# EDIpack/EDIpack

Measured on AMD Instinct MI355X. Metric: Lanczos H*v iterations/sec, largest (Nup,Ndw) sector, higher is better.
Workload: dtype f64

## Files before the change

edipack_amd/capi.py:

```python
from __future__ import annotations

import ctypes as C
import os

import numpy as np

HERE = os.path.dirname(os.path.abspath(__file__))
LIB_PATH = os.environ.get("EDIGPU_LIB", os.path.join(HERE, "lib", "libedigpu.so"))
HEADER_PATH = os.path.join(os.path.dirname(HERE), "include", "edigpu.h")

MAXORB = 5
MAXSUNDRY = 64
MAXBATH = 16


class EdigpuError(RuntimeError):
    """Raised when a C-ABI call returns non-zero (the Fortran shim does ``stop msg``)."""


class EdigpuModel(C.Structure):
    _fields_ = [
        ("ed_mode", C.c_int32), ("bath_type", C.c_int32),
        ("norb", C.c_int32), ("nbath", C.c_int32), ("nspin", C.c_int32), ("hfmode", C.c_int32),
        ("xmu", C.c_double),
        ("uloc", C.c_double * MAXORB),
        ("ust", C.c_double * (MAXORB * MAXORB)),
        ("jh", C.c_double * (MAXORB * MAXORB)),
        ("jx", C.c_double * (MAXORB * MAXORB)),
        ("jp", C.c_double * (MAXORB * MAXORB)),
        ("hloc", C.c_double * (2 * 2 * MAXORB * MAXORB * 2)),
        ("pair_field", C.c_double * MAXORB),
        ("be", C.c_double * (2 * MAXORB * MAXBATH)),
        ("bv", C.c_double * (2 * MAXORB * MAXBATH)),
        ("bd", C.c_double * (2 * MAXORB * MAXBATH)),
        ("bu", C.c_double * (2 * MAXORB * MAXBATH)),
        ("hb", C.c_double * (2 * 2 * MAXORB * MAXORB * MAXBATH * 2)),
        ("nph", C.c_int32), ("pad_", C.c_int32),
        ("w0_ph", C.c_double), ("a_ph", C.c_double),
        ("g_ph", C.c_double * (MAXORB * MAXORB)),
        ("spin_field", C.c_double * (MAXORB * 3)),
        ("exc_field", C.c_double * 4),
        ("nsundry", C.c_int32),
        ("pad2_", C.c_int32),
        ("sundry_op", C.c_int32 * (MAXSUNDRY * 8)),
        ("sundry_u", C.c_double * MAXSUNDRY),
    ]


_lib = None

_vp = C.c_void_p
_i64 = C.c_int64
_pi64 = C.POINTER(C.c_int64)
_pi32 = C.POINTER(C.c_int32)
_pd = C.POINTER(C.c_double)
_pint = C.POINTER(C.c_int)

SIGNATURES = {
    "edigpu_last_error": (C.c_char_p, []),
    "edigpu_version": (C.c_int, []),
    "edigpu_image_info": (C.c_int, [C.c_void_p, C.POINTER(C.c_int32)]),
    "edigpu_model_sizeof": (C.c_int64, []),
    "edigpu_device_count": (C.c_int, [_pint]),
    "edigpu_init": (C.c_int, [C.c_int]),
    "edigpu_normal_create": (C.c_int, [C.POINTER(_vp), _i64, _i64, _i64, _i64, _pd, _pi64, _pi32, _pd,
                                       _pi64, _pi32, _pd, _pi64, _pi32, _pd]),
    "edigpu_csr_create_d": (C.c_int, [C.POINTER(_vp), _i64, _i64, _i64, _pi64, _pi32, _pd]),
    "edigpu_csr_create_z": (C.c_int, [C.POINTER(_vp), _i64, _i64, _i64, _pi64, _pi32, _pd]),
    "edigpu_normal_build": (C.c_int, [C.POINTER(_vp), C.POINTER(EdigpuModel), C.c_int, C.c_int, _i64, _i64]),
    "edigpu_normal_build_z": (C.c_int, [C.POINTER(_vp), C.POINTER(EdigpuModel), C.c_int, C.c_int]),
    "edigpu_flat_build": (C.c_int, [C.POINTER(_vp), C.POINTER(EdigpuModel), C.c_int, _i64, _i64]),
    "edigpu_flat_build_jz": (C.c_int, [C.POINTER(_vp), C.POINTER(EdigpuModel), C.c_int, C.c_int, _i64, _i64]),
    "edigpu_direct_build_jz": (C.c_int, [C.POINTER(_vp), C.POINTER(EdigpuModel), C.c_int, C.c_int, _i64, _i64]),
    "edigpu_sector_map_jz": (C.c_int, [_vp, C.c_int, C.c_int, _pi32, _pi64]),
    "edigpu_direct_build": (C.c_int, [C.POINTER(_vp), C.POINTER(EdigpuModel), C.c_int, _i64, _i64]),
    "edigpu_sector_dim": (C.c_int, [C.POINTER(EdigpuModel), C.c_int, C.c_int, _pi64]),
    "edigpu_info": (C.c_int, [_vp, _pi64]),
    "edigpu_algorithmic_bytes": (C.c_int, [_vp, _pd, _pd]),
    "edigpu_normal_export": (C.c_int, [_vp, _pd, _pi64, _pi32, _pd, _pi64, _pi32, _pd, _pi64, _pi32, _pd]),
    "edigpu_csr_export": (C.c_int, [_vp, _pi64, _pi32, _pd]),
    "edigpu_apply_d": (C.c_int, [_vp, _i64, _pd, _pd]),
    "edigpu_apply_z": (C.c_int, [_vp, _i64, _pd, _pd]),
    "edigpu_apply_dev": (C.c_int, [_vp, _vp, _vp, _vp]),
    "edigpu_apply_local_dev": (C.c_int, [_vp, _vp, _vp, _vp]),
    "edigpu_apply_remote_dev": (C.c_int, [_vp, _vp, _vp, _vp]),
    "edigpu_normal_transpose_info": (C.c_int, [_vp, C.POINTER(C.c_int32)]),
    "edigpu_normal_apply_rows_dev": (C.c_int, [_vp, _i64, _i64, _vp, _vp, _vp]),
    "edigpu_normal_apply_cols_dev": (C.c_int, [_vp, _i64, _i64, _i64, C.c_int32, _vp, _vp, _vp]),
    "edigpu_transpose_pack": (C.c_int, [_i64, _i64, _i64, C.c_int32, _i64, C.c_int32, _vp, _vp, _vp]),
    "edigpu_transpose_unpack_add": (C.c_int, [_i64, _i64, _i64, C.c_int32, _i64, C.c_int32, _vp, _vp, _vp]),
    "edigpu_transpose_rotate_pack": (C.c_int, [C.c_int32, _i64, _i64, _i64, C.c_int32, _i64, C.c_int32, _vp, _vp, _vp,
                                               _vp, _vp]),
    "edigpu_transpose_unpack_add_dot2": (C.c_int, [_i64, _i64, _i64, C.c_int32, _i64, C.c_int32, _vp, _vp, _vp, _vp,
                                                   _vp, _vp, _vp]),
    "edigpu_lanczos_tridiag": (C.c_int, [_vp, _pd, C.c_int, _pd, _pd, C.c_double, _pint]),
    "edigpu_lanczos_eigh": (C.c_int, [_vp, C.c_int, C.c_double, C.c_int, _pd, _pd, _pd, _pint]),
    "edigpu_orbs_build": (C.c_int, [C.POINTER(_vp), C.POINTER(EdigpuModel), _pi32, _pi32]),
    "edigpu_orbs_build_rows": (C.c_int, [C.POINTER(_vp), C.POINTER(EdigpuModel), _pi32, _pi32, _i64, _i64]),
    "edigpu_orbs_create": (C.c_int, [C.POINTER(_vp), C.c_int, _pi64, _pd, _pi64, _pi32, _pd]),
    "edigpu_lanczos_eigh_multi": (C.c_int, [_vp, C.c_int, C.c_int, C.c_double, C.c_int, _vp, _pd, _vp,
                                            C.POINTER(C.c_int), C.POINTER(C.c_int)]),
    "edigpu_apply_op_normal": (C.c_int, [_vp, _vp, _vp, _vp, C.c_int, C.c_int, C.c_int, _vp]),
    "edigpu_apply_op_flat": (C.c_int, [_vp, _vp, _vp, _vp, C.c_int, C.c_int, C.c_int, _vp]),
    "edigpu_apply_cops_normal": (C.c_int, [_vp, _vp, _vp, _vp, C.c_int, _pd, _pi32, _pi32, _pi32, _vp]),
    "edigpu_lanczos_tridiag_dev": (C.c_int, [_vp, _vp, C.c_int, _pd, _pd, C.c_double, C.POINTER(C.c_int), _pd]),
    "edigpu_vec_work_doubles": (C.c_int, []),
    "edigpu_vec_rotate": (C.c_int, [_i64, _vp, _vp, _vp, _vp]),
    "edigpu_vec_add_dot": (C.c_int, [_i64, _vp, _vp, _vp, _vp, _vp, _vp]),
    "edigpu_vec_axpy_nrm2": (C.c_int, [_i64, _vp, _vp, _vp, _vp, _vp, _vp]),
    "edigpu_vec_scale": (C.c_int, [_i64, _vp, _vp, _vp]),
    "edigpu_vec_rotate_lazy": (C.c_int, [_i64, _vp, _vp, _vp, _vp]),
    "edigpu_vec_add_dot2": (C.c_int, [_i64, _vp, _vp, _vp, _vp, _vp, _vp]),
    "edigpu_time_apply": (C.c_int, [_vp, C.c_int, C.c_int, C.c_int, _pd]),
    "edigpu_lanczos_bench": (C.c_int, [_vp, C.c_int, C.c_int, _pd, _pd]),
# ... 102 lines not shown
```

edipack_amd/csrc/edigpu_capi.hip:

```cpp
#include <algorithm>
#include <chrono>
#include <cmath>
#include <cstdlib>
#include <cstring>
#include <map>
#include <memory>
#include <mutex>
#include <tuple>

#include "host_ib.hpp"
#include "host_sb.hpp"
#include "kernels.hpp"

namespace edigpu {

static thread_local std::string g_err;
static thread_local int g_device = 0;
void set_error(const std::string& msg) { g_err = msg; }

template <class T>
static int dev_upload(T** d, const T* h, size_t n) {
  *d = nullptr;
  if (n == 0) return 0;
  EDIGPU_HIP(hipMalloc((void**)d, n * sizeof(T)));
// ... 2058 lines not shown
    set_error("edigpu_sector_map: NULL argument");
    return 1;
  }
  std::vector<int32_t> st;
  std::string e = sector_map(*model, q1, q2, which, st);
  if (!e.empty()) {
    set_error(e);
    return 1;
  }
  if (map) {
    if (*n < (int64_t)st.size()) {
      set_error("edigpu_sector_map: output buffer too small");
      return 1;
    }
    std::copy(st.begin(), st.end(), map);
  }
  *n = (int64_t)st.size();
  return 0;
}

int edigpu_sector_map_jz(const edigpu_model* model, int ntot, int twojz, int32_t* map, int64_t* n) {
  if (!model || !n) {
    set_error("edigpu_sector_map_jz: NULL argument");
    return 1;
  }
  std::vector<int32_t> st;
  std::string e = sector_map_jz(*model, ntot, twojz, st);
  if (!e.empty()) {
    set_error(e);
    return 1;
  }
  if (map) {
    if (*n < (int64_t)st.size()) {
      set_error("edigpu_sector_map_jz: output buffer too small");
      return 1;
    }
    std::copy(st.begin(), st.end(), map);
  }
  *n = (int64_t)st.size();
  return 0;
}

int edigpu_image_info(edigpu_handle s, int32_t image[6]) {
  if (!s || !image || s->kind != 0) {
    set_error("edigpu_image_info: not a normal-mode handle");
    return 1;
  }
  image[0] = s->factored;
  image[1] = s->factored ? s->fac_nterms : 0;
  image[2] = s->factored ? s->fac_nimp : 0;
  image[3] = s->panel_mode;
  image[4] = s->ib ? kIbPanel : (s->blk_shift ? (1 << s->blk_shift) : 0);
  image[5] = s->ib ? (s->ib->sb ? (s->ib->sb->nhalf == 2 ? 4 : (s->ib->pr.on ? 5 : 3)) : s->ib->nhalf) : 0;
  return 0;
}

int edigpu_info(edigpu_handle s, int64_t info[10]) {
  if (!s || !info) {
    set_error("edigpu_info: NULL argument");
    return 1;
  }
  info[0] = s->dim;
  info[1] = s->nloc;
  info[2] = s->row_first;
  info[3] = s->is_complex;
  info[4] = s->kind;
  info[5] = s->dim_up;
  info[6] = s->dim_dw;
  if (s->kind == 0) {
    info[7] = s->h_up.nnz() + s->h_dw.nnz();
    info[8] = s->nd_nnz;
  } else if (s->kind == 4) {
    info[7] = s->sub_s->h_up.nnz() + s->sub_s->h_dw.nnz();
    info[8] = s->sub_s->nd_nnz;
  } else if (s->kind == 2) {
    info[7] = s->dir_nterms;
    info[8] = 0;
  } else if (s->kind == 3) {
    info[7] = 0;
    for (const HostCsr& f : s->h_orbs_fac) info[7] += f.nnz();
    info[8] = s->orbs.naxes;
  } else {
    info[7] = s->loc.nnz;
    info[8] = s->nonloc.nnz;
  }
  info[9] = s->device;
  return 0;
}

int edigpu_algorithmic_bytes(edigpu_handle s, double* bytes_hv, double* bytes_step) {
  if (!s) {
    set_error("edigpu_algorithmic_bytes: NULL handle");
    return 1;
  }
  double b = 0.0;
  const double sz = s->is_complex ? 16.0 : 8.0;
  if (s->kind == 4) {
    const edigpu_sector* r = s->sub_s;
    const double n = (double)s->nloc;
    b = 3.0 * sz * n;
    if (r->has_nd) b += (sz + 4.0) * (double)r->nd_nnz + 4.0 * (n + 1.0);
    b += (sz + 4.0) * (double)(r->h_up.nnz() + r->h_dw.nnz()) + 4.0 * (double)(r->dim_up + r->dim_dw + 2);
  } else if (s->kind == 0) {
    const double n = (double)s->nloc;
    b = 3.0 * sz * n;
    if (s->has_nd) b += (sz + 4.0) * (double)s->nd_nnz + 4.0 * (n + 1.0);
// ... 1179 lines not shown
```

edipack_amd/csrc/kernels.hpp:

```cpp
#pragma once
#include <functional>

#include "edigpu_internal.hpp"

namespace edigpu {

enum { SC_ALPHA = 0, SC_BETA = 1, SC_STOP = 2, SC_NDONE = 3, SC_NORM = 4, SC_THR = 5, SC_EXACT = 6, SC_AB = 8 };
constexpr int kRedBlocks = 1024;
constexpr int kMaxPartials = 1 << 16;

int ensure_dynamic_lds(const void* kernel, size_t bytes);
int resident_blocks(const void* kernel, int threads, size_t dyn_lds);
int device_cu_count();

int launch_normal(const edigpu_sector* s, const double* v_local, const double* v_full, double* hv,
                  int phase, hipStream_t st);
int normal_pick_rows_per_block(int64_t dim_up, int64_t dw_count);
bool normal_transposable(const edigpu_sector* s);
bool normal_transposable_el(const edigpu_sector* s);
int launch_normal_rows(const edigpu_sector* s, int64_t dw_first, int64_t dw_count, const double* v_rows,
                       double* hv_rows, hipStream_t st);
int launch_normal_cols(const edigpu_sector* s, int64_t col_first, int64_t ncol, int64_t stride, int halo,
                       const double* w, double* hv, hipStream_t st);
int launch_eph_scatter(int64_t n, const double* t, double* up, double c_up, double* dn, double c_dn, hipStream_t st);
int launch_deinterleave(int64_t n, const double* z, double* re, double* im, hipStream_t st);
int launch_combine_interleave(int64_t n, const double* yr, const double* yi, const double* t1, const double* t2,
                              double* z, hipStream_t st);
int launch_transpose_pack(int64_t dim_up, int64_t nrows, int64_t q, int world, int64_t pcol, int halo,
                          const double* v_rows, double* send, hipStream_t st);
int launch_transpose_unpack_add(int64_t dim_up, int64_t nrows, int64_t q, int world, int64_t pcol, int halo,
                                const double* recv, double* hv_rows, hipStream_t st);
bool normal_lanczos_fusable(const edigpu_sector* s);
int launch_normal_lanczos(const edigpu_sector* s, double* P, double* Q, const double* scal,
                          double* partial, int64_t partial_cap, bool first, bool lazy_axpy, hipStream_t st, int* npartial,
                          int nlanc = 0, bool* finalized = nullptr, double* X = nullptr, bool* in_x = nullptr);
int lz_finalize_alpha_beta(const double* P, const double* Q, int64_t n, double* partial, int np,
                           double* scal, int iter, int nlanc, hipStream_t st);
int lz_finalize_alpha(const double* partial, int np, double* scal, int iter, int nlanc, hipStream_t st);

int launch_csr(const DevCsr& a, int cplx, const double* x, double* y, int accumulate,
               hipStream_t st);
int launch_zero(double* y, int64_t n, hipStream_t st);

int launch_direct_lanczos(const edigpu_sector* s, const double* v_full, double* q, double* partial, int64_t cap, int* np,
                          const double* sig, hipStream_t st);
bool csr_lanczos_fusable(const DevCsr& a);
int launch_csr_lanczos(const DevCsr& a, int cplx, const double* x, double* y, double* partial, int64_t cap, int* np,
                       const double* sig, hipStream_t st);
int lz_rotate_lazy(double* P, double* Q, int64_t n, const double* scal, hipStream_t st);
int lz_next_vector(const double* P, const double* Q, double* X, int64_t n, const double* scal, bool lazy, hipStream_t st);
int launch_direct(const edigpu_sector* s, const double* v_full, double* hv, hipStream_t st);

int lz_norm_begin(double* vin, int64_t n, double* partial, double* scal, hipStream_t st);
int lz_rotate(double* vin, double* vout, int64_t n, const double* scal, hipStream_t st);
int lz_alpha(const double* vin, double* vout, const double* tmp, int64_t n, double* partial,
             double* scal, int iter, int nlanc, hipStream_t st);
int lz_beta(const double* vin, double* vout, int64_t n, double* partial, double* scal, int iter,
            int nlanc, hipStream_t st);
int lz_axpy_coef(double* acc, const double* vin, int64_t n, double coef, const double* scal,
                 int iter, hipStream_t st);
int lz_add_dot3(const double* P, double* Q, const double* tmp, int64_t n, const double* scal, double* partial, int* np,
                hipStream_t st);
int lz_fill_random(double* v, int64_t n, uint64_t seed, hipStream_t st);
int vec_to_blocked(const double* src, double* dst, int64_t dim_up, int64_t dim_dw, int shift, hipStream_t st);
int vec_from_blocked(const double* src, double* dst, int64_t dim_up, int64_t dim_dw, int shift, hipStream_t st);
int launch_normal_blocked(const edigpu_sector* s, const double* v, double* hv, hipStream_t st);
int vec_to_ib(const IbDev* ib, const double* src, double* dst, hipStream_t st);
int vec_from_ib(const IbDev* ib, const double* src, double* dst, hipStream_t st);
int launch_ib(const edigpu_sector* s, const double* v, double* hv, hipStream_t st);
int launch_ib_lanczos(const edigpu_sector* s, const double* P, double* Q, double* X, const double* scal, double* partial,
                      int64_t partial_cap, bool first, bool lazy_axpy, hipStream_t st, int* npartial);
int launch_sb(const edigpu_sector* s, const double* v, double* hv, hipStream_t st);
int launch_normal_rows_pos(const edigpu_sector* s, const double* P, double* Q, double* X, int what, const double* scal, hipStream_t st);
int launch_sb_lanczos(const edigpu_sector* s, const double* P, double* Q, double* X, const double* scal, double* partial,
                      int64_t partial_cap, bool first, bool lazy_axpy, hipStream_t st, int* npartial);
bool sb_shardable(const edigpu_sector* s);
int sb_shard_panels(const edigpu_sector* s, int world);
int sb_shard_to_panels(const edigpu_sector* s, const double* rows, double* dst, int64_t count, int64_t q, int world, hipStream_t st);
int sb_shard_from_panels_add(const edigpu_sector* s, const double* a, const double* b, double* rows, int64_t count, int64_t q, hipStream_t st);
int launch_sb_rows_shard(const edigpu_sector* s, int64_t row0, int64_t count, int64_t q, const double* v, double* hv, hipStream_t st);
int launch_sb_cols_shard(const edigpu_sector* s, int p0, int np, int64_t q, int npmax, const double* v, double* out, hipStream_t st);
int sb_nb0(int norb);
int sb_cols_waves();
int sb_cols_gs();
size_t sb_rows_lds(int nbw, int rimg_len, bool top = false);
// ... 78 lines not shown
```

edipack_amd/csrc/kernels_normal.hip:

```cpp
#include <cstdlib>
#include <string>

#include "kernels.hpp"
#include "normal_args.hpp"

namespace edigpu {



constexpr int kE = 4;

template <bool VEC>
__device__ inline void load4(const double* __restrict__ base, int64_t i0, const bool* ok, double* out) {
  if (VEC) {
    const double2 a = ok[0] ? *reinterpret_cast<const double2*>(base + i0) : make_double2(0.0, 0.0);
    const double2 b = ok[2] ? *reinterpret_cast<const double2*>(base + i0 + 2) : make_double2(0.0, 0.0);
    out[0] = a.x;
    out[1] = a.y;
    out[2] = b.x;
    out[3] = b.y;
  } else {
#pragma unroll
    for (int e = 0; e < kE; e++) out[e] = ok[e] ? base[i0 + e] : 0.0;
  }
}

typedef const double __attribute__((address_space(3))) lds_cdouble;
__device__ inline double lds_abs_read(uint32_t byte_addr) { return *reinterpret_cast<lds_cdouble*>(byte_addr); }

template <int NT, int TD, bool USE_LDS, bool LOCAL, bool ND, bool PACKED, bool VEC, bool HDF, int FUSE,
          bool SPLIT = false>
__global__ void __launch_bounds__(NT)
    normal_rows_kernel(NormalArgs a, const double* v_local, const double* __restrict__ v_full,
                       double* hv) {
  extern __shared__ double vs[];

  const int64_t DimUp = a.dim_up;
  const int bsh = a.blk_shift;
  const int64_t bps = a.blk_ps;
  auto vix = [&](int64_t row, int64_t col) -> int64_t {
    return bsh ? (col >> bsh) * bps + (row << bsh) + (col & (((int64_t)1 << bsh) - 1)) : row * DimUp + col;
  };
  const int64_t sf = SPLIT ? a.split_first : 0, sc = SPLIT ? a.split_count : DimUp;
  const int S = ((int)sc + 2) & ~1;
  const int rowB = S * 8;
  double* coef_s = vs + (USE_LDS ? TD * S : 0);
  const int64_t r0 = (int64_t)blockIdx.x * TD;
  const int tid = threadIdx.x;
  int nr = TD;
  if (r0 + nr > a.dw_count) nr = (int)(a.dw_count - r0);
  double beta = 0.0, ibeta = 1.0;
  if (FUSE != 0) {
    if (a.scal[SC_STOP] != 0.0) return;
    if (FUSE >= 2) {
// ... 303 lines not shown
    }
    case 102: {
      auto kern = normal_rows_kernel<NT, TD, USE_LDS, true, false, PACKED, VEC, HDF, 2>;
      if (ensure_dynamic_lds((const void*)kern, lds)) return 1;
      hipLaunchKernelGGL(kern, grid, block, lds, st, a, vl, vf, hv);
      break;
    }
    case 103: {
      auto kern = normal_rows_kernel<NT, TD, USE_LDS, true, false, PACKED, VEC, HDF, 3>;
      if (ensure_dynamic_lds((const void*)kern, lds)) return 1;
      hipLaunchKernelGGL(kern, grid, block, lds, st, a, vl, vf, hv);
      break;
    }
    case 4: EDIGPU_LAUNCH_ROWS(false, true, (size_t)0, false, false, false); break;
    default: set_error("launch_normal: bad term mask"); return 1;
  }
#undef EDIGPU_LAUNCH_ROWS
  EDIGPU_HIP(hipGetLastError());
  return 0;
}

template <int TD, bool USE_LDS>
static int launch_td(const NormalArgs& a, bool packed, bool hdf, const double* vl, const double* vf,
                     double* hv, int what, hipStream_t st) {
  const bool vec = (a.dim_up % 2) == 0;
  const bool big = TD == 1 && USE_LDS && (size_t)a.dim_up * sizeof(double) > 80 * 1024;
  constexpr int NTBIG = (TD == 1 && USE_LDS) ? 1024 : 512;
#define EDIGPU_TD(PK, VC)                                                                  \
  (big ? (hdf ? launch_te<NTBIG, TD, USE_LDS, PK, VC, true>(a, vl, vf, hv, what, st)       \
              : launch_te<NTBIG, TD, USE_LDS, PK, VC, false>(a, vl, vf, hv, what, st))     \
       : (hdf ? launch_te<512, TD, USE_LDS, PK, VC, true>(a, vl, vf, hv, what, st)         \
              : launch_te<512, TD, USE_LDS, PK, VC, false>(a, vl, vf, hv, what, st)))
  if (vec) return packed ? EDIGPU_TD(true, true) : EDIGPU_TD(false, true);
  return packed ? EDIGPU_TD(true, false) : EDIGPU_TD(false, false);
#undef EDIGPU_TD
}

template <bool VEC, bool HDF>
static int launch_split_t(const edigpu_sector* s, NormalArgs a, const double* vl, double* hv, hipStream_t st) {
  constexpr int NT = 1024;
  const int64_t part = (((a.dim_up + s->row_split - 1) / s->row_split) + 1) & ~(int64_t)1;
  auto kern = normal_rows_kernel<NT, 1, true, true, false, true, VEC, HDF, 0, true>;
  const size_t lds = (size_t)((part + 2) & ~(int64_t)1) * sizeof(double) + 128 * sizeof(double);
  if (ensure_dynamic_lds((const void*)kern, lds)) return 1;
  for (int64_t first = 0; first < a.dim_up; first += part) {
    a.split_first = first;
    a.split_count = std::min<int64_t>(part, a.dim_up - first);
    hipLaunchKernelGGL(kern, dim3((unsigned)a.dw_count), dim3(NT), lds, st, a, vl, nullptr, hv);
  }
  EDIGPU_HIP(hipGetLastError());
  return 0;
}

static int launch_rows(const edigpu_sector* s, const NormalArgs& a, const double* vl,
                       const double* vf, double* hv, int what, hipStream_t st) {
  const bool packed = s->up_ell.pk != nullptr;
  const bool hdf = s->factored != 0;
  if (s->row_split > 1 && what != 4) {
    if (what != 1 && what != 5) {
      set_error("launch_normal: fused Lanczos is not available for split rows");
      return 1;
    }
    const bool vec = (a.dim_up % 2) == 0;
    const int rc = vec ? (hdf ? launch_split_t<true, true>(s, a, vl, hv, st) : launch_split_t<true, false>(s, a, vl, hv, st))
                       : (hdf ? launch_split_t<false, true>(s, a, vl, hv, st) : launch_split_t<false, false>(s, a, vl, hv, st));
    if (rc || what == 1) return rc;
    return launch_td<1, false>(a, false, hdf, vl, vf, hv, 4, st);
  }
  switch (s->rows_per_block) {
    case 0: return launch_td<1, false>(a, packed, hdf, vl, vf, hv, what, st);
    case 1: return launch_td<1, true>(a, packed, hdf, vl, vf, hv, what, st);
    case 2: return launch_td<2, true>(a, packed, hdf, vl, vf, hv, what, st);
    case 4: return launch_td<4, true>(a, packed, hdf, vl, vf, hv, what, st);
    case 8: return launch_td<8, true>(a, packed, hdf, vl, vf, hv, what, st);
    default: set_error("launch_normal: bad rows_per_block"); return 1;
  }
}

static void fill_args(const edigpu_sector* s, NormalArgs& a) {
  a.dim_up = s->dim_up;
  a.dim_dw = s->dim_dw;
  a.dw_first = s->dw_first;
  a.dw_count = s->dw_count;
  a.hd = s->d_hd;
  a.eux = s->d_eux;
  a.ed = s->d_ed;
  a.impd = s->d_impd;
  a.ell_pk = s->up_ell.pk;
  a.ell_coef = s->up_ell.coef;
  a.ell_col = s->up_ell.col;
  a.ell_val = s->up_ell.val;
  a.ell_w = s->up_ell.width;
  a.ell_typed = s->up_ell.typed;
  a.ell_pitch = s->up_ell.pitch;
  a.dw_rowptr = s->dw.rowptr32;
  a.dw_col = s->dw.col;
  a.dw_val = s->dw.val;
  a.dw_maxrow = s->dw_maxrow;
  a.nd_rp32 = s->nd.rowptr32;
  a.nd_rp64 = s->nd.wide ? s->nd.rowptr64 : nullptr;
  a.nd_col = s->nd.col;
  a.nd_val = s->nd.val;
  a.has_nd = s->has_nd;
  a.nterms = s->factored ? s->fac_nterms : 0;
  a.nd_coef = s->d_ndcoef;
  a.jup = s->d_jup;
  a.jdw = s->d_jdw;
  a.panel_mode = s->panel_mode;
  a.tile_nchunks = s->tile_nchunks;
  a.tile_rows = s->tile_rows;
// ... 170 lines not shown
```

edipack_amd/hamiltonian.py:

```python
from __future__ import annotations

import ctypes as C
from dataclasses import dataclass, field

import numpy as np

from . import capi

ED_MODES = {"normal": 0, "superc": 1, "nonsu2": 2}
BATH_TYPES = {"normal": 0, "hybrid": 1, "replica": 2, "general": 3}


@dataclass
class ImpurityModel:
    ed_mode: str = "normal"
    bath_type: str = "normal"
    norb: int = 1
    nbath: int = 1
    nspin: int = 1
    hfmode: bool = True
    xmu: float = 0.0
    uloc: np.ndarray = field(default_factory=lambda: np.zeros(1))
    ust: np.ndarray | float = 0.0
    jh: np.ndarray | float = 0.0
# ... 194 lines not shown
            rp = np.asarray(rp, dtype=np.int64)
            rps.append(rp[1:] + base)
            base += int(rp[-1])
            cols.append(np.asarray(col, dtype=np.int32))
            vals.append(np.asarray(val, dtype=np.float64))
        rp = np.ascontiguousarray(np.concatenate(rps))
        col = np.ascontiguousarray(np.concatenate(cols)) if cols else np.zeros(0, np.int32)
        val = np.ascontiguousarray(np.concatenate(vals)) if vals else np.zeros(0, np.float64)
        h = C.c_void_p()
        capi.check(capi.lib().edigpu_orbs_create(C.byref(h), len(dims), capi.pi64(dims), capi.pd(hd), capi.pi64(rp),
                                                 capi.pi32(col), capi.pd(val)), "edigpu_orbs_create")
        return cls(h)

    @classmethod
    def normal_from_arrays(cls, dim_up, dim_dw, hd, up, dw, nd=None, dw_first=0, dw_count=None):
        if dw_count is None:
            dw_count = dim_dw
        hd = np.ascontiguousarray(hd, dtype=np.float64)
        ur, uc, uv = _csr_args(*up)
        dr, dc, dv = _csr_args(*dw)
        h = C.c_void_p()
        if nd is not None:
            nr, nc, nv = _csr_args(*nd)
            args = (capi.pi64(nr), capi.pi32(nc), capi.pd(nv))
        else:
            args = (None, None, None)
        capi.check(capi.lib().edigpu_normal_create(
            C.byref(h), dim_up, dim_dw, dw_first, dw_count, capi.pd(hd),
            capi.pi64(ur), capi.pi32(uc), capi.pd(uv), capi.pi64(dr), capi.pi32(dc), capi.pd(dv), *args),
            "edigpu_normal_create")
        return cls(h)

    @classmethod
    def csr_from_arrays(cls, rowptr, col, val, ncol_global=None, row_first=0):
        cplx = np.iscomplexobj(val)
        rowptr, col, val = _csr_args(rowptr, col, val, cplx)
        nrow = rowptr.shape[0] - 1
        if ncol_global is None:
            ncol_global = nrow
        h = C.c_void_p()
        fn = capi.lib().edigpu_csr_create_z if cplx else capi.lib().edigpu_csr_create_d
        capi.check(fn(C.byref(h), nrow, ncol_global, row_first, capi.pi64(rowptr), capi.pi32(col),
                      capi.pd(val.view(np.float64))), "edigpu_csr_create")
        return cls(h)

    def vecDim(self) -> int:
        return self.nloc

    def image_info(self):
        a = (C.c_int32 * 6)()
        capi.check(capi.lib().edigpu_image_info(self._h, a), "edigpu_image_info")
        return tuple(a)

    def algorithmic_bytes(self):
        a, b = C.c_double(), C.c_double()
        capi.check(capi.lib().edigpu_algorithmic_bytes(self._h, C.byref(a), C.byref(b)))
        return a.value, b.value

    def export_normal(self):
        nup_nnz_dw = None
        L = capi.lib()
        ur = np.zeros(self.dim_up + 1, np.int64)
        dr = np.zeros(self.dim_dw + 1, np.int64)
        nr = np.zeros(self.nloc + 1, np.int64)
        capi.check(L.edigpu_normal_export(self._h, None, capi.pi64(ur), None, None, capi.pi64(dr), None, None,
                                          capi.pi64(nr), None, None))
        hd = np.zeros(self.nloc)
        uc, uv = np.zeros(ur[-1], np.int32), np.zeros(ur[-1])
        dc, dv = np.zeros(dr[-1], np.int32), np.zeros(dr[-1])
        nc, nv = np.zeros(nr[-1], np.int32), np.zeros(nr[-1])
        capi.check(L.edigpu_normal_export(self._h, capi.pd(hd), None, capi.pi32(uc), capi.pd(uv), None,
                                          capi.pi32(dc), capi.pd(dv), None, capi.pi32(nc), capi.pd(nv)))
        del nup_nnz_dw
        return hd, (ur, uc, uv), (dr, dc, dv), (nr, nc, nv)

    def export_csr(self):
        L = capi.lib()
        rp = np.zeros(self.nloc + 1, np.int64)
        nnz = self.nnz_a + self.nnz_b
        col = np.zeros(nnz, np.int32)
        val = np.zeros(nnz, self.dtype)
        capi.check(L.edigpu_csr_export(self._h, capi.pi64(rp), capi.pi32(col), capi.pd(val.view(np.float64))))
        return rp, col, val

    def apply(self, v: np.ndarray, hv: np.ndarray | None = None) -> np.ndarray:
        v = np.ascontiguousarray(v, dtype=self.dtype)
        if hv is None:
            hv = np.empty_like(v)
        fn = capi.lib().edigpu_apply_z if self.is_complex else capi.lib().edigpu_apply_d
        capi.check(fn(self._h, v.shape[0], capi.pd(v.view(np.float64)), capi.pd(hv.view(np.float64))),
                   "edigpu_apply")
        return hv

    def apply_dev(self, v_full_ptr: int, hv_ptr: int, stream: int = 0) -> None:
        capi.check(capi.lib().edigpu_apply_dev(self._h, v_full_ptr, hv_ptr, stream if stream else None), "edigpu_apply_dev")

    def apply_local_dev(self, v_local_ptr: int, hv_ptr: int, stream: int = 0) -> None:
        capi.check(capi.lib().edigpu_apply_local_dev(self._h, v_local_ptr, hv_ptr, stream if stream else None),
                   "edigpu_apply_local_dev")

    def apply_remote_dev(self, v_full_ptr: int, hv_ptr: int, stream: int = 0) -> None:
        capi.check(capi.lib().edigpu_apply_remote_dev(self._h, v_full_ptr, hv_ptr, stream if stream else None),
                   "edigpu_apply_remote_dev")

    def apply_cops_to(self, dst: "SectorHamiltonian", v_src_ptr: int, v_dst_ptr: int, coefs, creates, iorbs, ispins,
                      stream: int = 0) -> None:
# ... 213 lines not shown
```

include/edigpu.h:

```cpp
#ifndef EDIGPU_H
#define EDIGPU_H

#include <stdint.h>

#ifdef __cplusplus
extern "C" {
#endif

#define EDIGPU_MAXORB 5
#define EDIGPU_MAXSUNDRY 64
#define EDIGPU_MAXBATH 16

typedef struct edigpu_sector *edigpu_handle;

const char *edigpu_last_error(void);
int edigpu_version(void);
int64_t edigpu_model_sizeof(void);
int edigpu_device_count(int *count);
int edigpu_init(int device);

int edigpu_normal_create(edigpu_handle *h, int64_t dim_up, int64_t dim_dw, int64_t dw_first,
                         int64_t dw_count, const double *hd, const int64_t *up_rowptr,
                         const int32_t *up_col, const double *up_val, const int64_t *dw_rowptr,
                         const int32_t *dw_col, const double *dw_val, const int64_t *nd_rowptr,
// ... 13 lines not shown
  int32_t hfmode;
  double xmu;
  double uloc[EDIGPU_MAXORB];
  double ust[EDIGPU_MAXORB * EDIGPU_MAXORB];
  double jh[EDIGPU_MAXORB * EDIGPU_MAXORB];
  double jx[EDIGPU_MAXORB * EDIGPU_MAXORB];
  double jp[EDIGPU_MAXORB * EDIGPU_MAXORB];
  double hloc[2 * 2 * EDIGPU_MAXORB * EDIGPU_MAXORB * 2];
  double pair_field[EDIGPU_MAXORB];
  double be[2 * EDIGPU_MAXORB * EDIGPU_MAXBATH];
  double bv[2 * EDIGPU_MAXORB * EDIGPU_MAXBATH];
  double bd[2 * EDIGPU_MAXORB * EDIGPU_MAXBATH];
  double bu[2 * EDIGPU_MAXORB * EDIGPU_MAXBATH];
  double hb[2 * 2 * EDIGPU_MAXORB * EDIGPU_MAXORB * EDIGPU_MAXBATH * 2];
  int32_t nph;
  int32_t pad_;
  double w0_ph, a_ph;
  double g_ph[EDIGPU_MAXORB * EDIGPU_MAXORB];
  double spin_field[EDIGPU_MAXORB * 3];
  double exc_field[4];
  int32_t nsundry;
  int32_t pad2_;
  int32_t sundry_op[EDIGPU_MAXSUNDRY * 8];
  double sundry_u[EDIGPU_MAXSUNDRY];
} edigpu_model;

int edigpu_normal_build(edigpu_handle *h, const edigpu_model *model, int nup, int ndw,
                        int64_t dw_first, int64_t dw_count);
int edigpu_normal_build_z(edigpu_handle *h, const edigpu_model *model, int nup, int ndw);
int edigpu_flat_build(edigpu_handle *h, const edigpu_model *model, int sector, int64_t row_first,
                      int64_t row_count);

int edigpu_flat_build_jz(edigpu_handle *h, const edigpu_model *model, int ntot, int twojz, int64_t row_first,
                         int64_t row_count);
int edigpu_direct_build_jz(edigpu_handle *h, const edigpu_model *model, int ntot, int twojz, int64_t row_first,
                           int64_t row_count);
int edigpu_sector_map_jz(const edigpu_model *model, int ntot, int twojz, int32_t *map, int64_t *n);

int edigpu_direct_build(edigpu_handle *h, const edigpu_model *model, int sector, int64_t row_first,
                        int64_t row_count);

int edigpu_orbs_build(edigpu_handle *h, const edigpu_model *model, const int32_t *nups, const int32_t *ndws);
int edigpu_orbs_build_rows(edigpu_handle *h, const edigpu_model *model, const int32_t *nups, const int32_t *ndws,
                           int64_t row_first, int64_t row_count);
int edigpu_orbs_create(edigpu_handle *h, int naxes, const int64_t *dims, const double *hd,
                       const int64_t *fac_rowptr, const int32_t *fac_col, const double *fac_val);

int edigpu_sector_dim(const edigpu_model *model, int q1, int q2, int64_t *dim);

int edigpu_sector_map(const edigpu_model *model, int q1, int q2, int which, int32_t *map, int64_t *n);

int edigpu_info(edigpu_handle h, int64_t info[10]);
int edigpu_image_info(edigpu_handle h, int32_t image[6]);
int edigpu_algorithmic_bytes(edigpu_handle h, double *bytes_hv, double *bytes_lanczos_step);
int edigpu_normal_export(edigpu_handle h, double *hd, int64_t *up_rowptr, int32_t *up_col,
                         double *up_val, int64_t *dw_rowptr, int32_t *dw_col, double *dw_val,
                         int64_t *nd_rowptr, int32_t *nd_col, double *nd_val);
int edigpu_csr_export(edigpu_handle h, int64_t *rowptr, int32_t *col, double *val);

int edigpu_apply_d(edigpu_handle h, int64_t nloc, const double *v_host, double *hv_host);
int edigpu_apply_z(edigpu_handle h, int64_t nloc, const double *v_host, double *hv_host);

int edigpu_apply_dev(edigpu_handle h, const void *v_full_dev, void *hv_dev, void *stream);
int edigpu_apply_local_dev(edigpu_handle h, const void *v_local_dev, void *hv_dev, void *stream);
int edigpu_apply_remote_dev(edigpu_handle h, const void *v_full_dev, void *hv_dev, void *stream);

int edigpu_normal_transpose_info(edigpu_handle h, int32_t *halo);
int edigpu_normal_apply_rows_dev(edigpu_handle h, int64_t dw_first, int64_t dw_count, const void *v_rows_dev,
                                 void *hv_rows_dev, void *stream);
int edigpu_normal_apply_cols_dev(edigpu_handle h, int64_t col_first, int64_t col_count, int64_t row_stride,
                                 int32_t halo, const void *w_cols_dev, void *hv_cols_dev, void *stream);
int edigpu_transpose_pack(int64_t dim_up, int64_t nrows, int64_t q, int32_t world, int64_t pcol, int32_t halo,
                          const void *v_rows_dev, void *send_dev, void *stream);
int edigpu_transpose_unpack_add(int64_t dim_up, int64_t nrows, int64_t q, int32_t world, int64_t pcol,
                                int32_t halo, const void *recv_dev, void *hv_rows_dev, void *stream);
int edigpu_transpose_rotate_pack(int32_t first, int64_t dim_up, int64_t nrows, int64_t q, int32_t world,
                                 int64_t pcol, int32_t halo, void *vin_dev, void *vout_dev, const void *ab_dev,
                                 void *send_dev, void *stream);
int edigpu_transpose_unpack_add_dot2(int64_t dim_up, int64_t nrows, int64_t q, int32_t world, int64_t pcol,
                                     int32_t halo, const void *vin_dev, void *vout_dev, const void *tmp_dev,
                                     const void *back_dev, void *out2_dev, void *work_dev, void *stream);

int edigpu_lanczos_tridiag(edigpu_handle h, const double *vin_host, int nlanc, double *alanc,
                           double *blanc, double threshold, int *niter_done);
int edigpu_lanczos_eigh_multi(edigpu_handle h, int neigen, int ncv, double tol, int maxrestart, const double *v0,
                              double *evals, double *evecs, int *nconv, int *nmatvec);

int edigpu_apply_op_normal(edigpu_handle src, edigpu_handle dst, const double *v_src_dev, double *v_dst_dev,
                           int iorb, int ispin, int create, void *stream);
int edigpu_apply_cops_normal(edigpu_handle src, edigpu_handle dst, const double *v_src_dev, double *v_dst_dev,
                             int nops, const double *coef, const int32_t *create, const int32_t *iorb,
                             const int32_t *ispin, void *stream);
int edigpu_apply_op_flat(edigpu_handle src, edigpu_handle dst, const double *v_src_dev, double *v_dst_dev,
                         int iorb, int ispin, int create, void *stream);
int edigpu_apply_cops_flat(edigpu_handle src, edigpu_handle dst, const double *v_src_dev, double *v_dst_dev, int nops,
                           const double *coef_re_im, const int32_t *create, const int32_t *iorb, const int32_t *ispin,
                           void *stream);
int edigpu_lanczos_tridiag_dev(edigpu_handle h, const double *vin_dev, int nlanc, double *alanc, double *blanc,
                               double threshold, int *niter_done, double *norm2);

int edigpu_lanczos_eigh(edigpu_handle h, int nitermax, double tol, int check_every,
                        const double *v0_host, double *eval, double *evec_host,
                        int *niter_done);

int edigpu_vec_work_doubles(void);
int edigpu_vec_rotate(int64_t n, double *vin_dev, double *vout_dev, const double *beta2_dev, void *stream);
// ... 67 lines not shown
```

Baseline: 6365.

## Add persistent row kernel with LDS double-buffered staging via loader waves

Adds a persistent kernel for the normal-mode row apply. Each workgroup owns a contiguous range of down-rows. Two dedicated loader waves prefetch the next row of the vector into a double-buffered LDS slot with global_load_lds, while compute waves hold the packed ELL offsets and signs in registers and gather from LDS. The kernel also fuses the Lanczos scaling and alpha/beta updates, and the kernel is selected automatically when the sector fits the constraints. It is meant to hide global-load latency and avoid reloading the ELL structure for every row. In exchange it uses fixed large workgroups, a barrier per row, and tight eligibility limits.

Result: faster. 6485, median of 6 (+1.9%).

```diff
diff --git a/edipack_amd/capi.py b/edipack_amd/capi.py
--- a/edipack_amd/capi.py
+++ b/edipack_amd/capi.py
@@ -60,6 +60,7 @@
     "edigpu_last_error": (C.c_char_p, []),
     "edigpu_version": (C.c_int, []),
     "edigpu_image_info": (C.c_int, [C.c_void_p, C.POINTER(C.c_int32)]),
+    "edigpu_rows_kernel": (C.c_int, [C.c_void_p, C.POINTER(C.c_int32)]),
     "edigpu_model_sizeof": (C.c_int64, []),
     "edigpu_device_count": (C.c_int, [_pint]),
     "edigpu_init": (C.c_int, [C.c_int]),
diff --git a/edipack_amd/csrc/edigpu_capi.hip b/edipack_amd/csrc/edigpu_capi.hip
--- a/edipack_amd/csrc/edigpu_capi.hip
+++ b/edipack_amd/csrc/edigpu_capi.hip
@@ -2134,6 +2134,15 @@
   image[3] = s->panel_mode;
   image[4] = s->ib ? kIbPanel : (s->blk_shift ? (1 << s->blk_shift) : 0);
   image[5] = s->ib ? (s->ib->sb ? (s->ib->sb->nhalf == 2 ? 4 : (s->ib->pr.on ? 5 : 3)) : s->ib->nhalf) : 0;
+  return 0;
+}
+
+int edigpu_rows_kernel(edigpu_handle s, int32_t* kind) {
+  if (!s || !kind || s->kind != 0) {
+    set_error("edigpu_rows_kernel: not a normal-mode handle");
+    return 1;
+  }
+  *kind = normal_rows_persistent(s) ? 1 : 0;
   return 0;
 }
 
diff --git a/edipack_amd/csrc/kernels.hpp b/edipack_amd/csrc/kernels.hpp
--- a/edipack_amd/csrc/kernels.hpp
+++ b/edipack_amd/csrc/kernels.hpp
@@ -31,6 +31,7 @@
 int launch_transpose_unpack_add(int64_t dim_up, int64_t nrows, int64_t q, int world, int64_t pcol, int halo,
                                 const double* recv, double* hv_rows, hipStream_t st);
 bool normal_lanczos_fusable(const edigpu_sector* s);
+bool normal_rows_persistent(const edigpu_sector* s);
 int launch_normal_lanczos(const edigpu_sector* s, double* P, double* Q, const double* scal,
                           double* partial, int64_t partial_cap, bool first, bool lazy_axpy, hipStream_t st, int* npartial,
                           int nlanc = 0, bool* finalized = nullptr, double* X = nullptr, bool* in_x = nullptr);
diff --git a/edipack_amd/csrc/kernels_normal.hip b/edipack_amd/csrc/kernels_normal.hip
--- a/edipack_amd/csrc/kernels_normal.hip
+++ b/edipack_amd/csrc/kernels_normal.hip
@@ -1,5 +1,6 @@
 #include <cstdlib>
 #include <string>
+#include <type_traits>
 
 #include "kernels.hpp"
 #include "normal_args.hpp"
@@ -409,10 +410,231 @@
   return 0;
 }
 
+constexpr int kPrNT = 1024;
+constexpr int kPrLoaders = 2;
+constexpr int kPrMaxCols = (kPrNT / 64 - kPrLoaders) * 256 - 1;
+constexpr int kPrSlots = 16;
+constexpr uint32_t kPrRowB = ((kPrMaxCols >> 7) + 1) * 1024;
+constexpr uint32_t kPrCoefB = 128 * sizeof(double);
+constexpr int kPrRows = 256;
+
+__host__ __device__ constexpr uint32_t pr_meta_off(int fuse) { return kPrCoefB + 2u * (fuse >= 2 ? 2u : 1u) * kPrRowB; }
+__host__ __device__ constexpr uint32_t pr_lds_bytes(int fuse) { return pr_meta_off(fuse) + kPrRows * 12u; }
+
+__device__ inline void pr_barrier() {
+  asm volatile("s_waitcnt lgkmcnt(0)" ::: "memory");
+  __builtin_amdgcn_s_barrier();
+  asm volatile("" ::: "memory");
+}
+
+template <int FUSE>
+__global__ void __launch_bounds__(kPrNT) __attribute__((amdgpu_waves_per_eu(4, 4))) normal_rows_persistent_kernel(NormalArgs a, const double* v_local, double* hv) {
+  extern __shared__ double vs[];
+  constexpr int kV = FUSE >= 2 ? 2 : 1;
+  const int DimUp = (int)a.dim_up;
+  const int64_t bps = a.blk_ps;
+  const int tid = threadIdx.x, lane = tid & 63;
+  const int wave = __builtin_amdgcn_readfirstlane(tid >> 6);
+  const int ncw = (int)(blockDim.x >> 6) - kPrLoaders;
+  const bool loader = wave >= ncw;
+  double beta = 0.0, ibeta = 1.0;
+  if (FUSE != 0) {
+    if (a.scal[SC_STOP] != 0.0) return;
+    if (FUSE >= 2) {
+      beta = a.scal[SC_BETA];
+      ibeta = 1.0 / beta;
+    }
+  }
+  const double alpha = (FUSE == 3) ? a.scal[SC_ALPHA] : 0.0;
+  const double* __restrict__ v_src = (FUSE >= 2) ? hv : v_local;
+  double* const pout = a.xout ? a.xout : const_cast<double*>(v_local);
+  if ((uint32_t)(uintptr_t)(__attribute__((address_space(3))) double*)vs != 0u) __builtin_trap();
+  if (tid < 128) vs[tid] = a.ell_coef[tid];
+  const int64_t rbeg = (int64_t)blockIdx.x * a.dw_count / gridDim.x;
+  const int64_t rend = (int64_t)(blockIdx.x + 1) * a.dw_count / gridDim.x;
+
+  typedef __attribute__((address_space(3))) void lds_void;
+  typedef __attribute__((address_space(1))) const void glb_void;
+  const int npc = (DimUp + 127) >> 7;
+  const int zw = (DimUp >> 7) % kPrLoaders;
+  auto stage = [&](int64_t r, int s) {
+    const int lw = wave - ncw;
+#pragma unroll
+    for (int j = 0; j < kV; j++) {
+      const double* src = (j == 0 ? v_src : v_local) + (r << 7) + 2 * lane;
+      const uint32_t dst = kPrCoefB + (uint32_t)(s * kV + j) * kPrRowB;
+      for (int p = lw; p < npc; p += kPrLoaders)
+        __builtin_amdgcn_global_load_lds((glb_void*)(src + p * bps), (lds_void*)((char*)vs + dst + p * 1024), 16, 0, 0);
+    }
+  };
+  auto land = [&](int s) {
+    __builtin_amdgcn_s_waitcnt(0x0F70);
+    if (wave - ncw == zw && lane == 0) vs[(kPrCoefB + (uint32_t)s * kV * kPrRowB) / 8 + DimUp] = 0.0;
+  };
+
+  const int col0 = 4 * tid;
+  const bool act = !loader && col0 < DimUp;
+  bool ok[kE];
+#pragma unroll
+  for (int e = 0; e < kE; e++) ok[e] = col0 + e < DimUp;
+  const int kw4 = (a.ell_w + 3) & ~3;
+  uint2 pk[kPrSlots];
+#pragma unroll
+  for (int k = 0; k < kPrSlots; k++) {
+    const int kc = k < a.ell_w ? k : a.ell_w - 1;
+    const uint4 w = act ? *reinterpret_cast<const uint4*>(a.ell_pk + (int64_t)kc * a.ell_pitch + col0) : make_uint4(0, 0, 0, 0);
+    auto pair = [](uint32_t lo, uint32_t hi) {
+      return (lo & 0x7FFFu) | ((lo >> 31) << 15) | ((hi & 0x7FFFu) << 16) | (hi & 0x80000000u);
+    };
+    pk[k] = make_uint2(pair(w.x, w.y), pair(w.z, w.w));
+  }
+  double* const med = vs + pr_meta_off(FUSE) / 8;
+  int* const mim = reinterpret_cast<int*>(med + kPrRows);
+  auto eux4 = [&](int64_t r, double* q) {
+    const int i = (int)((r < rend ? r : rend - 1) - rbeg);
+    load4<false>(a.eux, (int64_t)mim[i] * DimUp + col0, ok, q);
+  };
+  auto edr = [&](int64_t r) { return med[(int)((r < rend ? r : rend - 1) - rbeg)]; };
+  if (loader) {
+    stage(rbeg, 0);
+    land(0);
+  } else {
+    for (int i = tid; i < (int)(rend - rbeg); i += ncw * 64) {
+      med[i] = a.ed[a.dw_first + rbeg + i];
+      mim[i] = a.impd[a.dw_first + rbeg + i];
+    }
+  }
+  pr_barrier();
+  double hc[kE], eq[kE];
+  if (!loader) {
+    eux4(rbeg, hc);
+    const double e0 = edr(rbeg);
+#pragma unroll
+    for (int e = 0; e < kE; e++) hc[e] += e0;
+  }
+
+  auto step = [&](auto S, int64_t r) {
+    constexpr int s = decltype(S)::value;
+    constexpr uint32_t xb = kPrCoefB + (uint32_t)s * kV * kPrRowB;
+    constexpr uint32_t pb = xb + kPrRowB;
+    double* const xs = vs + xb / 8;
+    const double* const ps = vs + pb / 8;
+    if (loader) {
+      const bool more = r + 1 < rend;
+      if (more) stage(r + 1, s ^ 1);
+      if (FUSE >= 2) pr_barrier();
+      land(s ^ 1);
+      pr_barrier();
+      return;
+    }
+    eux4(r + 1, eq);
+#pragma unroll
+    for (int k = 0; k < kPrSlots; k++) asm volatile("" : "+v"(pk[k].x), "+v"(pk[k].y));
+    if (FUSE >= 2) {
+#pragma unroll
+      for (int e = 0; e < kE; e++) {
+        double t = xs[col0 + e];
+        if (FUSE == 3) t -= alpha * ps[col0 + e];
+        t *= ibeta;
+        xs[col0 + e] = ok[e] ? t : 0.0;
+      }
+      pr_barrier();
+    }
+    if (act) {
+      double acc[kE];
+#pragma unroll
+      for (int e = 0; e < kE; e++) acc[e] = hc[e] * (ok[e] ? xs[col0 + e] : 0.0);
+#pragma unroll
+      for (int k0 = 0; k0 < kPrSlots; k0 += 4) {
+        if (k0 >= kw4) break;
+        double xg[4][kE];
+#pragma unroll
+        for (int u = 0; u < 4; u++)
+#pragma unroll
+          for (int e = 0; e < kE; e++) {
+            const uint32_t w = (e & 2) ? pk[k0 + u].y : pk[k0 + u].x;
+            const uint32_t off = (e & 1) ? (w >> 16) & 0x7FFFu : w & 0x7FFFu;
+            const uint32_t sg = (e & 1) ? w & 0x80000000u : (w << 16) & 0x80000000u;
+            const double x = lds_abs_read(xb + off);
+            xg[u][e] = __hiloint2double(__double2hiint(x) ^ (int)sg, __double2loint(x));
+          }
+#pragma unroll
+        for (int u = 0; u < 4; u++) {
+          const double tk = vs[k0 + u];
+#pragma unroll
+          for (int e = 0; e < kE; e++) acc[e] = fma(tk, xg[u][e], acc[e]);
+        }
+      }
+      const double e1 = edr(r + 1);
+#pragma unroll
+      for (int e = 0; e < kE; e++) {
+        hc[e] = eq[e] + e1;
+        asm volatile("" : "+v"(hc[e])::"memory");
+      }
+      const int64_t o = ((int64_t)(col0 >> 7)) * bps + (r << 7) + (col0 & 127);
+      if (FUSE >= 2) {
+#pragma unroll
+        for (int e = 0; e < kE; e++) acc[e] -= beta * ps[col0 + e];
+        if (ok[3]) {
+          *reinterpret_cast<double2*>(pout + o) = make_double2(xs[col0], xs[col0 + 1]);
+          *reinterpret_cast<double2*>(pout + o + 2) = make_double2(xs[col0 + 2], xs[col0 + 3]);
+        } else {
+#pragma unroll
+          for (int e = 0; e < kE; e++)
+            if (ok[e]) pout[o + e] = xs[col0 + e];
+        }
+      }
+      if (ok[3]) {
+        *reinterpret_cast<double2*>(hv + o) = make_double2(acc[0], acc[1]);
+        *reinterpret_cast<double2*>(hv + o + 2) = make_double2(acc[2], acc[3]);
+      } else {
+#pragma unroll
+        for (int e = 0; e < kE; e++)
+          if (ok[e]) hv[o + e] = acc[e];
+      }
+    }
+    pr_barrier();
+  };
+  for (int64_t r = rbeg; r < rend; r += 2) {
+    step(std::integral_constant<int, 0>(), r);
+    if (r + 1 < rend) step(std::integral_constant<int, 1>(), r + 1);
+  }
+}
+
+bool normal_rows_persistent(const edigpu_sector* s) {
+  return s->kind == 0 && s->blk_shift == 7 && s->factored && s->row_split == 1 && s->rows_per_block >= 1 &&
+         s->up_ell.pk != nullptr && s->up_ell.typed && s->up_ell.width >= 1 && s->up_ell.width <= kPrSlots &&
+         s->dim_up <= kPrMaxCols && s->dw_count > 0;
+}
+
+static int launch_rows_persistent(const NormalArgs& a, const double* vl, double* hv, int what, hipStream_t st) {
+  const int ncw = (int)(a.dim_up / 256) + 1;
+  const int64_t nwg = std::max<int64_t>(std::min<int64_t>(device_cu_count(), a.dw_count), (a.dw_count + kPrRows - 1) / kPrRows);
+  const dim3 grid((unsigned)nwg), block((unsigned)(ncw + kPrLoaders) * 64);
+  auto go = [&](auto kern, int fuse) -> int {
+    if (ensure_dynamic_lds((const void*)kern, pr_lds_bytes(fuse))) return 1;
+    hipLaunchKernelGGL(kern, grid, block, pr_lds_bytes(fuse), st, a, vl, hv);
+    return 0;
+  };
+  int rc;
+  switch (what) {
+    case 1: rc = go(normal_rows_persistent_kernel<0>, 0); break;
+    case 101: rc = go(normal_rows_persistent_kernel<1>, 1); break;
+    case 102: rc = go(normal_rows_persistent_kernel<2>, 2); break;
+    case 103: rc = go(normal_rows_persistent_kernel<3>, 3); break;
+    default: set_error("launch_rows_persistent: bad term mask"); return 1;
+  }
+  if (rc) return rc;
+  EDIGPU_HIP(hipGetLastError());
+  return 0;
+}
+
 static int launch_rows(const edigpu_sector* s, const NormalArgs& a, const double* vl,
                        const double* vf, double* hv, int what, hipStream_t st) {
   const bool packed = s->up_ell.pk != nullptr;
   const bool hdf = s->factored != 0;
+  if (a.blk_shift == 7 && (what == 1 || (what >= 101 && what <= 103)) && normal_rows_persistent(s))
+    return launch_rows_persistent(a, vl, hv, what, st);
   if (s->row_split > 1 && what != 4) {
     if (what != 1 && what != 5) {
       set_error("launch_normal: fused Lanczos is not available for split rows");
diff --git a/edipack_amd/hamiltonian.py b/edipack_amd/hamiltonian.py
--- a/edipack_amd/hamiltonian.py
+++ b/edipack_amd/hamiltonian.py
@@ -270,6 +270,11 @@
         capi.check(capi.lib().edigpu_image_info(self._h, a), "edigpu_image_info")
         return tuple(a)
 
+    def rows_kernel(self) -> int:
+        k = C.c_int32()
+        capi.check(capi.lib().edigpu_rows_kernel(self._h, C.byref(k)), "edigpu_rows_kernel")
+        return k.value
+
     def algorithmic_bytes(self):
         a, b = C.c_double(), C.c_double()
         capi.check(capi.lib().edigpu_algorithmic_bytes(self._h, C.byref(a), C.byref(b)))
diff --git a/include/edigpu.h b/include/edigpu.h
--- a/include/edigpu.h
+++ b/include/edigpu.h
@@ -89,6 +89,7 @@
 
 int edigpu_info(edigpu_handle h, int64_t info[10]);
 int edigpu_image_info(edigpu_handle h, int32_t image[6]);
+int edigpu_rows_kernel(edigpu_handle h, int32_t *kind);
 int edigpu_algorithmic_bytes(edigpu_handle h, double *bytes_hv, double *bytes_lanczos_step);
 int edigpu_normal_export(edigpu_handle h, double *hd, int64_t *up_rowptr, int32_t *up_col,
                          double *up_val, int64_t *dw_rowptr, int32_t *dw_col, double *dw_val,
```
